# alphacep/vosk-tts

Hardware: NVIDIA H100
Metric: audio samples/sec @22.05kHz, 128-phoneme utterance (higher is better)
Workload: dtype fp32 (flow/decoder convs + attention: bf16 hi+lo split x3 MMAs on wgmma, fp32 accumulate; rest fp32 FFMA)

## Files before the change

### vosk_tts_b200/csrc/conv_tc.cuh

```cuda
#pragma once
#include <type_traits>
#include <cuda.h>
#include <cuda_bf16.h>
#include <cuda_runtime.h>
#include <stdint.h>
#include "wgmma.cuh"

namespace vtts {

constexpr int TC_BM = 128;
constexpr int TC_BK = 64;
#ifndef VTTS_TC_AST64
#define VTTS_TC_AST64 3
#endif
#ifndef VTTS_TC_WST64
#define VTTS_TC_WST64 4
#endif
#ifndef VTTS_TC_AST128
#define VTTS_TC_AST128 3
#endif
#ifndef VTTS_TC_WST128
#define VTTS_TC_WST128 4
#endif
template <int BN> constexpr int tc_ast() { return BN == 64 ? VTTS_TC_AST64 : VTTS_TC_AST128; }
template <int BN> constexpr int tc_wst() { return BN == 64 ? VTTS_TC_WST64 : VTTS_TC_WST128; }
constexpr int TC_CWG = 2;
constexpr int TC_THREADS = TC_CWG * 128 + 32;
constexpr int TC_MAXP = 4;

enum : int { TCE_RELU = 1, TCE_GATE = 2 };

struct TcProblemBase {
  CUtensorMap a_hi, a_lo, w_hi, w_lo;
  __nv_bfloat16* p_mid;
  const float* bias;
  const float* cond;
  const float* res;
  float* y;
  __nv_bfloat16* p_hi;
  __nv_bfloat16* p_lo;
  int cond_ld, ldr, roff, ldy, yoff, ldp, poff;
  int Cin, Cout, k, dil, pad;
  int out_mul, out_add;
  int in_extra, out_seq_extra;
  int epi;
  float alpha, pl_slope;
  int split;
  int cl0;
};
struct TcProblem : TcProblemBase {
  CUtensorMap a_mid, w_mid;
};

struct TcBatchScalars {
  int n;
  int rmul;
  int tall;
  int a_bytes;
  int baseoff;
  int cn;
  int wpre;
  int np;
  int ast, wst;
  int dbgskip;
  int wmc;
  int persist;
  int gx, gy, gz;
  int split;
  int mixed;
  int nb;
  unsigned long long* dbg;
};
template <class PT, int MP = TC_MAXP>
struct TcBatchT : TcBatchScalars {
  PT p[MP];
};
using TcBatch = TcBatchT<TcProblem>;
template <int MP>
inline TcBatchT<TcProblemBase, MP> tc_lite(const TcBatch& tb) {
  TcBatchT<TcProblemBase, MP> l;
  static_cast<TcBatchScalars&>(l) = tb;
  for (int i = 0; i < MP; ++i) l.p[i] = tb.p[i];
  return l;
}
__device__ __forceinline__ unsigned long long gtimer() {
  unsigned long long t;
  asm volatile("mov.u64 %0, %globaltimer;" : "=l"(t));
  return t;
}
#define TC_STAMP(i) do { if (tb.dbg && blockIdx.x == 0 && blockIdx.y == 0 && blockIdx.z == 0) tb.dbg[i] = gtimer(); } while (0)

__device__ __forceinline__ void tma_load_2d(void* dst, const CUtensorMap* map, int c0, int c1, uint64_t* bar) {
  asm volatile(
      "cp.async.bulk.tensor.2d.shared::cluster.global.mbarrier::complete_tx::bytes [%0], [%1, {%3, %4}], [%2];" ::"r"(smem_u32(dst)),
      "l"(reinterpret_cast<uint64_t>(map)), "r"(smem_u32(bar)), "r"(c0), "r"(c1)
      : "memory");
}
__device__ __forceinline__ void tma_load_2d_mc(void* dst, const CUtensorMap* map, int c0, int c1, uint64_t* bar, uint16_t mask) {
  asm volatile(
      "cp.async.bulk.tensor.2d.shared::cluster.global.mbarrier::complete_tx::bytes.multicast::cluster [%0], [%1, {%3, %4}], [%2], %5;" ::"r"(
          smem_u32(dst)),
      "l"(reinterpret_cast<uint64_t>(map)), "r"(smem_u32(bar)), "r"(c0), "r"(c1), "h"(mask)
      : "memory");
}
__device__ __forceinline__ uint32_t cluster_rank() {
  uint32_t r;
  asm volatile("mov.u32 %0, %%cluster_ctarank;" : "=r"(r));
  return r;
}
__device__ __forceinline__ void mbar_arrive_remote(uint64_t* bar, uint32_t rank) {
  uint32_t ra;
  asm volatile("mapa.shared::cluster.u32 %0, %1, %2;" : "=r"(ra) : "r"(smem_u32(bar)), "r"(rank));
  asm volatile("mbarrier.arrive.release.cluster.shared::cluster.b64 _, [%0];" ::"r"(ra) : "memory");
}
__device__ __forceinline__ void tc_release(uint64_t* bar, int n) {
  if (n > 1) {
    for (int r = 0; r < n; ++r) mbar_arrive_remote(bar, (uint32_t)r);
  } else {
    mbar_arrive(bar);
  }
}

__device__ __forceinline__ float tc_bias(const TcProblemBase& P, int b, int c) {
  float bv = P.bias[c];
  if (P.cond) bv += P.cond[(long)b * P.cond_ld + c];
  return bv;
}
__device__ __forceinline__ void tc_epi_pair(const TcProblemBase& P, int b, long orow, int c, float v0, float v1, int dbgskip) {
  const bool gate = (P.epi & TCE_GATE) != 0;
  float u[2];
  int oc, nout;
  if (gate) {
    oc = c >> 1;
    if (oc >= (P.Cout >> 1)) return;
    nout = 1;
    const float a = v0 + tc_bias(P, b, c), s = v1 + tc_bias(P, b, c + 1);
    u[0] = tanhf(a) * (1.f / (1.f + expf(-s)));
    u[1] = 0.f;
  } else {
    oc = c;
    if (oc >= P.Cout) return;
    nout = min(2, P.Cout - oc);
    u[0] = v0 + tc_bias(P, b, c);
    u[1] = nout > 1 ? v1 + tc_bias(P, b, c + 1) : 0.f;
  }
  const bool relu = (P.epi & TCE_RELU) != 0;
#pragma unroll
  for (int e = 0; e < 2; ++e) {
    float q = u[e];
    if (relu) q = fmaxf(q, 0.f);
    u[e] = q * P.alpha;
  }
  if (P.res && !(dbgskip & 4)) {
    const float* rp = P.res + orow * (long)P.ldr + P.roff + oc;
    if (nout == 2 && ((P.ldr | P.roff | oc) & 1) == 0) {
      const float2 q2 = *reinterpret_cast<const float2*>(rp);
      u[0] += q2.x; u[1] += q2.y;
    } else {
      for (int e = 0; e < nout; ++e) u[e] += rp[e];
    }
  }
  if (dbgskip & 1) return;
  if (P.y) {
    float* yr = P.y + orow * (long)P.ldy + P.yoff + oc;
    if (nout == 2 && ((P.ldy | P.yoff | oc) & 1) == 0) *reinterpret_cast<float2*>(yr) = make_float2(u[0], u[1]);
    else for (int e = 0; e < nout; ++e) yr[e] = u[e];
  }
  if (P.p_hi) {
    const long po = orow * (long)P.ldp + P.poff + oc;
    __align__(4) __nv_bfloat16 hb[2], mb[2], lb[2];
#pragma unroll
    for (int e = 0; e < 2; ++e) {
      float q = u[e];
      q = q > 0.f ? q : q * P.pl_slope;
      if (P.p_mid) split_bf16_3(q, hb[e], mb[e], lb[e]);
      else split_bf16(q, hb[e], lb[e]);
    }
    if (nout == 2 && ((P.ldp | P.poff | oc) & 1) == 0) {
      *reinterpret_cast<uint32_t*>(P.p_hi + po) = *reinterpret_cast<const uint32_t*>(hb);
      *reinterpret_cast<uint32_t*>(P.p_lo + po) = *reinterpret_cast<const uint32_t*>(lb);
      if (P.p_mid) *reinterpret_cast<uint32_t*>(P.p_mid + po) = *reinterpret_cast<const uint32_t*>(mb);
    } else {
      for (int e = 0; e < nout; ++e) {
        P.p_hi[po + e] = hb[e]; P.p_lo[po + e] = lb[e];
        if (P.p_mid) P.p_mid[po + e] = mb[e];
      }
    }
  }
}

template <int BN>
constexpr int tc_smem_bytes(int a_bytes, int np = 2, int ast = tc_ast<BN>(), int wst = tc_wst<BN>()) {
  return ast * np * a_bytes + wst * np * BN * TC_BK * 2 + 1024  + 256 ;
}
constexpr int TC_MAXST = 4;

struct TcTile {
  int pi;
  int b, co0, t0, sp;
  int s;
  int t0u;
  bool valid;
};

template <int BN, bool MIXED, class PT, int MP>
__device__ __forceinline__ void conv_tc_body(const TcBatchT<PT, MP>& tb, const int* __restrict__ lens, const int* __restrict__ offs) {
  constexpr bool HAS_MID = std::is_same<PT, TcProblem>::value;
  constexpr int B_BYTES = BN * TC_BK * 2;
  constexpr int NACC = BN / 2;
  const int TC_AST = tb.ast, TC_WST = tb.wst, NP = HAS_MID ? tb.np : 2;
  PDL_LAUNCH();
  if (threadIdx.x == 0) TC_STAMP(0);
  const int S = tb.split;
  const bool persist = tb.persist != 0;
  const int A_BYTES = tb.a_bytes;
  const bool tall = tb.tall != 0;
  const int wmc = persist ? tb.wmc : 1;
  const uint32_t wrank = wmc > 1 ? cluster_rank() : 0u;
  const int gxu = (tb.gx + wmc - 1) / wmc;
  const int ntiles = persist ? gxu * tb.gy * tb.gz : 1;
  const int tstride = persist ? (int)gridDim.x / wmc : 1;
  const int tile0 = persist ? (int)blockIdx.x / wmc : 0;
  auto decode_mixed = [&](int g) {
    const int ci = (int)blockIdx.z / S, rank = (int)blockIdx.z - ci * S;
    int pi = 0;
    while (pi + 1 < tb.n && ci >= tb.p[pi + 1].cl0) ++pi;
    const int s = tb.p[pi].split, gyp = (tb.p[pi].Cout + BN - 1) / BN;
    if (g < 0) g = rank / s;
    const int tile = (ci - tb.p[pi].cl0) * (S / s) + g;
    TcTile t;
    t.pi = pi;
    t.s = s;
    t.sp = rank % s;
    t.t0 = (tile % tb.gx) * TC_BM;
    t.t0u = t.t0;
    t.co0 = ((tile / tb.gx) % gyp) * BN;
    t.b = tile / (tb.gx * gyp);
    t.valid = t.b < tb.nb;
    return t;
  };
  auto decode = [&](int tile) {
    if constexpr (MIXED) { if (tb.mixed) return decode_mixed(-1); }
    int bx, by, bz, bxu;
    if (persist) {
      bxu = tile % gxu;
      const int r = tile / gxu;
      by = r % tb.gy;
      bz = r / tb.gy;
      bx = bxu * wmc + (int)wrank;
    } else {
      bx = blockIdx.x; by = blockIdx.y; bz = blockIdx.z;
      bxu = bx;
    }
    TcTile t;
    t.t0u = bxu * wmc * TC_BM;
    const int zi = bz / S;
    t.s = S;
    t.sp = bz - zi * S;
    t.pi = zi % tb.n;
    t.b = zi / tb.n;
    t.co0 = by * BN;
    t.t0 = bx * TC_BM;
    t.valid = t.co0 < tb.p[t.pi].Cout;
    return t;
  };

  extern __shared__ uint8_t tc_smem_raw[];
  uint8_t* smem = reinterpret_cast<uint8_t*>((reinterpret_cast<uintptr_t>(tc_smem_raw) + 1023) & ~(uintptr_t)1023);
  uint8_t* smem_w = smem + TC_AST * NP * A_BYTES;
  uint64_t* a_full = reinterpret_cast<uint64_t*>(smem_w + TC_WST * NP * B_BYTES);
  uint64_t* a_empty = a_full + TC_MAXST;
  uint64_t* w_full = a_empty + TC_MAXST;
  uint64_t* w_empty = w_full + TC_MAXST;

  const int warp = threadIdx.x >> 5, lane = threadIdx.x & 31;
  const bool producer = warp == TC_CWG * 4;
  const TcTile first = decode(tile0);
  const int cn = tb.cn;

  if (producer && lane == 0) {
    for (int s = 0; s < TC_AST; ++s) { mbar_init(&a_full[s], 1); mbar_init(&a_empty[s], (uint32_t)(cn * TC_CWG)); }
    for (int s = 0; s < TC_WST; ++s) { mbar_init(&w_full[s], 1); mbar_init(&w_empty[s], (uint32_t)(wmc * TC_CWG)); }
    asm volatile("fence.mbarrier_init.release.cluster;" ::: "memory");
    for (int q = 0; q < (persist ? tb.n : 1); ++q) {
      const PT& Q = tb.p[persist ? q : first.pi];
      asm volatile("prefetch.tensormap [%0];" ::"l"(reinterpret_cast<uint64_t>(&Q.a_hi)) : "memory");
      asm volatile("prefetch.tensormap [%0];" ::"l"(reinterpret_cast<uint64_t>(&Q.a_lo)) : "memory");
      asm volatile("prefetch.tensormap [%0];" ::"l"(reinterpret_cast<uint64_t>(&Q.w_hi)) : "memory");
      asm volatile("prefetch.tensormap [%0];" ::"l"(reinterpret_cast<uint64_t>(&Q.w_lo)) : "memory");
      if constexpr (HAS_MID) {
        if (NP == 3) {
          asm volatile("prefetch.tensormap [%0];" ::"l"(reinterpret_cast<uint64_t>(&Q.a_mid)) : "memory");
          asm volatile("prefetch.tensormap [%0];" ::"l"(reinterpret_cast<uint64_t>(&Q.w_mid)) : "memory");
        }
      }
    }
  }
  __syncthreads();
  const uint32_t crank = cn > 1 ? cluster_rank() : 0u;
  const uint16_t cmask = (uint16_t)((1u << cn) - 1u);
  if (cn > 1 || wmc > 1) cluster_sync_all();
  int w_pre = 0;
  auto issue_w = [&](const PT& P, int co0, int c, int j, int wst) {
    uint8_t* wb = smem_w + wst * NP * B_BYTES;
    mbar_expect_tx(&w_full[wst], NP * B_BYTES);
    if (wmc > 1) {
      const int half = (int)wrank * (BN / 2);
      tma_load_2d_mc(wb + half * 128, &P.w_hi, c * TC_BK, j * P.Cout + co0 + half, &w_full[wst], (uint16_t)3);
      tma_load_2d_mc(wb + B_BYTES + half * 128, &P.w_lo, c * TC_BK, j * P.Cout + co0 + half, &w_full[wst], (uint16_t)3);
      return;
    }
    tma_load_2d(wb, &P.w_hi, c * TC_BK, j * P.Cout + co0, &w_full[wst]);
    tma_load_2d(wb + B_BYTES, &P.w_lo, c * TC_BK, j * P.Cout + co0, &w_full[wst]);
    if constexpr (HAS_MID) { if (NP == 3) tma_load_2d(wb + 2 * B_BYTES, &P.w_mid, c * TC_BK, j * P.Cout + co0, &w_full[wst]); }
  };
  if (!persist && first.valid) {
    const PT& P = tb.p[first.pi];
    const int nsteps_all = (P.Cin / TC_BK) * P.k;
    const int s_beg = (int)((long)nsteps_all * first.sp / first.s), s_end = (int)((long)nsteps_all * (first.sp + 1) / first.s);
    const bool peek_active = first.t0 < lens[first.b] * tb.rmul + P.in_extra;
    w_pre = (tb.wpre && peek_active) ? min(TC_WST, s_end - s_beg) : 0;
    if (producer && lane == 0) {
      int c = s_beg / P.k, j = s_beg - c * P.k;
      for (int i = 0; i < w_pre; ++i) {
        issue_w(P, first.co0, c, j, i);
        if (++j == P.k) { j = 0; ++c; }
      }
    }
  }
  PDL_WAIT();
  if (threadIdx.x == 0) TC_STAMP(1);
  bool any_active = false;

  if (producer) {
    if (lane == 0) {
      int ast = 0, a_use = 0, wst = 0, w_use = 0;
      for (int tile = tile0; tile < ntiles; tile += tstride) {
        const TcTile T = persist ? decode(tile) : first;
        if (!T.valid) continue;
        const PT& P = tb.p[T.pi];
        const int L = lens[T.b] * tb.rmul + P.in_extra;
        if (T.t0u >= L) {
          for (int i = 0; i < w_pre; ++i) mbar_wait(&w_full[i], 0);
          continue;
        }
        any_active = true;
        const long in_base = (long)offs[T.b] * tb.rmul + (long)T.b * P.in_extra;
        const int nsteps_all = (P.Cin / TC_BK) * P.k;
        const int s_beg = (int)((long)nsteps_all * T.sp / T.s), s_end = (int)((long)nsteps_all * (T.sp + 1) / T.s);
        const int a_per = tall ? P.k : 1;
        const uint32_t a_tx = (uint32_t)NP * (uint32_t)(tall ? (TC_BM + (P.k - 1) * P.dil) : TC_BM) * 128u;
        int c = s_beg / P.k, j = s_beg - c * P.k;
        int a_cnt = 0;
        for (int s = s_beg; s < s_end; ++s) {
          const int ls = s - s_beg;
          if (a_cnt == 0) {
            if (a_use > 0) mbar_wait(&a_empty[ast], (a_use - 1) & 1);
            uint8_t* ab = smem + ast * NP * A_BYTES;
            mbar_expect_tx(&a_full[ast], a_tx);
            const int row = (int)in_base + T.t0 - P.pad + (tall ? 0 : j * P.dil);
            if (cn > 1) {
              const int slice = TC_BM / cn;
              const int soff = (int)crank * slice;
              tma_load_2d_mc(ab + soff * 128, &P.a_hi, c * TC_BK, row + soff, &a_full[ast], cmask);
              tma_load_2d_mc(ab + A_BYTES + soff * 128, &P.a_lo, c * TC_BK, row + soff, &a_full[ast], cmask);
            } else {
              tma_load_2d(ab, &P.a_hi, c * TC_BK, row, &a_full[ast]);
              tma_load_2d(ab + A_BYTES, &P.a_lo, c * TC_BK, row, &a_full[ast]);
              if constexpr (HAS_MID) { if (NP == 3) tma_load_2d(ab + 2 * A_BYTES, &P.a_mid, c * TC_BK, row, &a_full[ast]); }
            }
            if (++ast == TC_AST) { ast = 0; ++a_use; }
          }
          if (++a_cnt == a_per) a_cnt = 0;
          if (ls >= w_pre) {
            if (w_use > 0) mbar_wait(&w_empty[wst], (w_use - 1) & 1);
            issue_w(P, T.co0, c, j, wst);
          }
          if (++wst == TC_WST) { wst = 0; ++w_use; }
          if (++j == P.k) { j = 0; ++c; }
          if (ls == 0) TC_STAMP(2);
        }
        w_pre = 0;
        TC_STAMP(3);
      }
    }
    any_active = __shfl_sync(0xffffffffu, (int)any_active, 0) != 0;
  } else {
    const int wg = warp >> 2;
    const int g = lane >> 2, q4 = lane & 3;
    const int rbase = wg * 64 + (warp & 3) * 16 + g;
    const bool leader = (threadIdx.x & 127) == 0;
    int ast = 0, a_use = 0, wst = 0, w_use = 0;
    for (int tile = tile0; tile < ntiles; tile += tstride) {
      const TcTile T = persist ? decode(tile) : first;
      if (!T.valid) continue;
      const PT& P = tb.p[T.pi];
      const int L = lens[T.b] * tb.rmul + P.in_extra;
      if (T.t0u >= L) continue;
      any_active = true;
      const int nsteps_all = (P.Cin / TC_BK) * P.k;
      const int s_beg = (int)((long)nsteps_all * T.sp / T.s), s_end = (int)((long)nsteps_all * (T.sp + 1) / T.s);
      const int a_per = tall ? P.k : 1;
      float acc[NACC];
#pragma unroll
      for (int i = 0; i < NACC; ++i) acc[i] = 0.f;
      int j = s_beg % P.k;
      int a_cnt = 0;
      int prev_w = -1, prev_a = -1;
      for (int s = s_beg; s < s_end; ++s) {
        const int ls = s - s_beg;
        if (a_cnt == 0) mbar_wait(&a_full[ast], a_use & 1);
        mbar_wait(&w_full[wst], w_use & 1);
        if (ls == 0 && threadIdx.x == 0) TC_STAMP(4);
        const uint32_t abase = smem_u32(smem + ast * NP * A_BYTES) + (uint32_t)(wg * 64 * 128) + (tall ? (uint32_t)(j * P.dil) * 128u : 0u);
        const uint32_t wbase = smem_u32(smem_w + wst * NP * B_BYTES);
        const uint64_t ahi = gmma_desc_sw128(abase, tb.baseoff), alo = gmma_desc_sw128(abase + A_BYTES, tb.baseoff);
        const uint64_t bhi = gmma_desc_sw128(wbase), blo = gmma_desc_sw128(wbase + B_BYTES);
        auto mma = [&](uint64_t da, uint64_t db) {
          if constexpr (BN == 128) wgmma_ss_n128(acc, da, db);
          else wgmma_ss_n64(acc, da, db);
        };
        wgmma_fence();
        if (tb.dbgskip & 2) {
        } else if (NP == 3) {
          const uint64_t ami = gmma_desc_sw128(abase + 2 * A_BYTES, tb.baseoff), bmi = gmma_desc_sw128(wbase + 2 * B_BYTES);
#pragma unroll
          for (int kk = 0; kk < TC_BK / 16; ++kk) {
            const uint64_t adv = (uint64_t)((kk * 32) >> 4);
            mma(ahi + adv, blo + adv);
            mma(alo + adv, bhi + adv);
            mma(ami + adv, bmi + adv);
            mma(ami + adv, bhi + adv);
            mma(ahi + adv, bmi + adv);
            mma(ahi + adv, bhi + adv);
          }
        } else {
#pragma unroll
          for (int kk = 0; kk < TC_BK / 16; ++kk) {
            const uint64_t adv = (uint64_t)((kk * 32) >> 4);
            mma(alo + adv, bhi + adv);
            mma(ahi + adv, blo + adv);
            mma(ahi + adv, bhi + adv);
          }
        }
        wgmma_commit();
        wgmma_wait<1>();
        wgmma_touch<NACC>(acc);
        if (leader) {
          if (prev_w >= 0) tc_release(&w_empty[prev_w], wmc);
          if (prev_a >= 0) tc_release(&a_empty[prev_a], cn);
        }
        prev_w = wst;
        prev_a = -1;
        if (++wst == TC_WST) { wst = 0; ++w_use; }
        if (++a_cnt == a_per) {
          prev_a = ast;
          a_cnt = 0;
          if (++ast == TC_AST) { ast = 0; ++a_use; }
        }
        if (++j == P.k) j = 0;
      }
      wgmma_wait<0>();
      wgmma_touch<NACC>(acc);
      if (leader) {
        if (prev_w >= 0) tc_release(&w_empty[prev_w], wmc);
        if (prev_a >= 0) tc_release(&a_empty[prev_a], cn);
      }
      if (threadIdx.x == 0) TC_STAMP(5);
      const int b = T.b, co0 = T.co0;
      const long out_base = (long)offs[b] * tb.rmul * P.out_mul + (long)b * P.out_seq_extra;
      long orow[2];
      bool rowok[2];
#pragma unroll
      for (int h = 0; h < 2; ++h) {
        const int t = T.t0 + rbase + 8 * h;
        rowok[h] = t < L;
        orow[h] = out_base + (long)t * P.out_mul + P.out_add;
      }
      if (T.s == 1) {
#pragma unroll
        for (int jn = 0; jn < BN / 8; ++jn) {
          const int c = co0 + jn * 8 + 2 * q4;
#pragma unroll
          for (int h = 0; h < 2; ++h)
            if (rowok[h]) tc_epi_pair(P, b, orow[h], c, acc[4 * jn + 2 * h], acc[4 * jn + 2 * h + 1], tb.dbgskip);
        }
      } else {
        const int W = BN / T.s, sp = T.sp, g0 = MIXED ? (int)blockIdx.z % S - sp : 0;
        float* stage = reinterpret_cast<float*>(smem);
        cluster_sync_all();
#pragma unroll
        for (int jn = 0; jn < BN / 8; ++jn) {
          const int cc = jn * 8 + 2 * q4;
          const int qo = cc / W;
#pragma unroll
          for (int h = 0; h < 2; ++h) {
            uint32_t ra;
            asm volatile("mapa.shared::cluster.u32 %0, %1, %2;" : "=r"(ra) : "r"(smem_u32(stage + ((size_t)sp * TC_BM + rbase + 8 * h) * W + (cc - qo * W))), "r"(g0 + qo));
            asm volatile("st.shared::cluster.v2.f32 [%0], {%1, %2};" ::"r"(ra), "f"(acc[4 * jn + 2 * h]), "f"(acc[4 * jn + 2 * h + 1]) : "memory");
          }
        }
        cluster_sync_all();
#pragma unroll 1
        for (int u = 0; u < W / 4; ++u) {
          const int cw = 2 * q4 + 8 * (u >> 1), row = rbase + 8 * (u & 1), t = T.t0 + row;
          float v0 = 0.f, v1 = 0.f;
          for (int src = 0; src < T.s; ++src) {
            const float2 p2 = *reinterpret_cast<const float2*>(stage + ((size_t)src * TC_BM + row) * W + cw);
            v0 += p2.x; v1 += p2.y;
          }
          if (t < L) tc_epi_pair(P, b, out_base + (long)t * P.out_mul + P.out_add, co0 + sp * W + cw, v0, v1, tb.dbgskip);
        }
      }
    }
  }
  if (first.s > 1) {
    bool cl_active = any_active;
    if (MIXED && tb.mixed)
      for (int g = 0; g < S / first.s; ++g) {
        const TcTile u = decode_mixed(g);
        if (u.valid && u.t0 < lens[u.b] * tb.rmul + tb.p[u.pi].in_extra) cl_active = true;
      }
    if (cl_active && (producer || !any_active)) {
      __syncwarp();
      cluster_sync_all();
      cluster_sync_all();
    }
  }
  if (threadIdx.x == 0) TC_STAMP(7);
  __syncthreads();
  if (cn > 1 || wmc > 1) cluster_sync_all();
  if (threadIdx.x == 0) TC_STAMP(8);
}

template <int BN, bool DYN, int MP = TC_MAXP>
__global__ void __launch_bounds__(TC_THREADS, 1)
conv_tc_kernel(const __grid_constant__ TcBatchT<std::conditional_t<DYN, TcProblem, TcProblemBase>, MP> tb, const int* __restrict__ lens,
               const int* __restrict__ offs) {
  conv_tc_body<BN, true>(tb, lens, offs);
}
template <int BN>
__global__ void __launch_bounds__(TC_THREADS, 1)
conv_tc_persist_kernel(const __grid_constant__ TcBatch tb, const int* __restrict__ lens, const int* __restrict__ offs) {
  conv_tc_body<BN, false>(tb, lens, offs);
}

constexpr int EW_THREADS = 256;
constexpr int EW_ROWS = 16;

__global__ void __launch_bounds__(EW_THREADS)
split_planes_kernel(const float* __restrict__ x, int ldx, __nv_bfloat16* __restrict__ hi, __nv_bfloat16* __restrict__ lo,
                    int ldp, int C, float slope, int reflect, int rmul, const int* __restrict__ lens,
                    const int* __restrict__ offs) {
  PDL_LAUNCH();
  PDL_WAIT();
  const int b = blockIdx.y;
  const int Lphys = lens[b] * rmul;
  const int L = Lphys + (reflect ? 1 : 0);
  const int p0 = blockIdx.x * EW_ROWS;
  if (p0 >= L) return;
  const int nq = C >> 2;
  const int nrow = min(EW_ROWS, L - p0);
  const long base = (long)offs[b] * rmul;
  for (int u = threadIdx.x; u < nrow * nq; u += EW_THREADS) {
    const int r = u / nq, c = (u - r * nq) << 2;
    const int p = p0 + r;
    const int pr = reflect ? (p == 0 ? 1 : p - 1) : p;
    const long irow = base + pr;
    const long orow = base + (reflect ? b : 0) + p;
    const float4 v = *reinterpret_cast<const float4*>(x + irow * ldx + c);
    const float f[4] = {v.x, v.y, v.z, v.w};
    __align__(8) __nv_bfloat16 hb[4], lb[4];
#pragma unroll
    for (int i = 0; i < 4; ++i) {
      const float q = f[i] > 0.f ? f[i] : f[i] * slope;
      split_bf16(q, hb[i], lb[i]);
    }
    *reinterpret_cast<uint2*>(hi + orow * ldp + c) = *reinterpret_cast<const uint2*>(hb);
    *reinterpret_cast<uint2*>(lo + orow * ldp + c) = *reinterpret_cast<const uint2*>(lb);
  }
}

__global__ void __launch_bounds__(EW_THREADS)
mrf_mean_planes_kernel(const float* __restrict__ a, const float* __restrict__ b2, const float* __restrict__ c3, int n,
                       float* __restrict__ out, __nv_bfloat16* __restrict__ hi, __nv_bfloat16* __restrict__ lo, int C,
                       float slope, int reflect, int rmul, const int* __restrict__ lens, const int* __restrict__ offs) {
  PDL_LAUNCH();
  PDL_WAIT();
  const int b = blockIdx.y;
  const int Lphys = lens[b] * rmul;
  const int L = Lphys + (reflect ? 1 : 0);
  const int p0 = blockIdx.x * EW_ROWS;
  if (p0 >= L) return;
  const int nq = C >> 2;
  const int nrow = min(EW_ROWS, L - p0);
  const long base = (long)offs[b] * rmul;
  const float d = (float)n;
  for (int u = threadIdx.x; u < nrow * nq; u += EW_THREADS) {
    const int r = u / nq, c = (u - r * nq) << 2;
    const int p = p0 + r;
    const int pr = reflect ? (p == 0 ? 1 : p - 1) : p;
    const long irow = base + pr;
    const long orow = base + (reflect ? b : 0) + p;
    float4 s = *reinterpret_cast<const float4*>(a + irow * C + c);
    if (n > 1) { const float4 q = *reinterpret_cast<const float4*>(b2 + irow * C + c); s.x += q.x; s.y += q.y; s.z += q.z; s.w += q.w; }
    if (n > 2) { const float4 q = *reinterpret_cast<const float4*>(c3 + irow * C + c); s.x += q.x; s.y += q.y; s.z += q.z; s.w += q.w; }
    s.x /= d; s.y /= d; s.z /= d; s.w /= d;
    if (out && (!reflect || p >= 1)) *reinterpret_cast<float4*>(out + irow * C + c) = s;
    const float f[4] = {s.x, s.y, s.z, s.w};
    __align__(8) __nv_bfloat16 hb[4], lb[4];
#pragma unroll
    for (int i = 0; i < 4; ++i) {
      const float q = f[i] > 0.f ? f[i] : f[i] * slope;
      split_bf16(q, hb[i], lb[i]);
    }
    *reinterpret_cast<uint2*>(hi + orow * C + c) = *reinterpret_cast<const uint2*>(hb);
    *reinterpret_cast<uint2*>(lo + orow * C + c) = *reinterpret_cast<const uint2*>(lb);
  }
}

}
```

Measured before the change: 17.38 million.

## Prefetch epilogue bias/residual loads and overlap them with final wgmma wait

The epilogue is restructured around a precomputed TcEpi descriptor and per-column loads. Bias, cond and residual values for the first column are issued before the final wgmma wait, and each later column's inputs are prefetched one step ahead so global-load latency overlaps compute and stores. The split (s==1) and cluster-reduction paths now share one column loop, which walks columns by shifting the accumulator array each iteration. This adds register pressure and runtime-indexed or non-unrolled loops (unroll 1) that may cost instruction overhead.

```diff
diff --git a/vosk_tts_b200/csrc/conv_tc.cuh b/vosk_tts_b200/csrc/conv_tc.cuh
--- a/vosk_tts_b200/csrc/conv_tc.cuh
+++ b/vosk_tts_b200/csrc/conv_tc.cuh
@@ -121,69 +121,128 @@
   }
 }
 
-__device__ __forceinline__ float tc_bias(const TcProblemBase& P, int b, int c) {
-  float bv = P.bias[c];
-  if (P.cond) bv += P.cond[(long)b * P.cond_ld + c];
-  return bv;
-}
-__device__ __forceinline__ void tc_epi_pair(const TcProblemBase& P, int b, long orow, int c, float v0, float v1, int dbgskip) {
-  const bool gate = (P.epi & TCE_GATE) != 0;
+
+struct TcEpi {
+  const float* bias;
+  const float* cond;
+  const float* res;
+  float* y;
+  __nv_bfloat16 *p_hi, *p_lo, *p_mid;
+  int ldr, roff, ldy, yoff, ldp, poff;
+  int ncol;
+  float alpha, pl_slope;
+  bool gate, relu, store;
+};
+template <class PT>
+__device__ __forceinline__ TcEpi tc_epi(const PT& P, int b, int dbgskip) {
+  TcEpi E;
+  E.bias = P.bias;
+  E.cond = P.cond ? P.cond + (long)b * P.cond_ld : nullptr;
+  E.res = (dbgskip & 4) ? nullptr : P.res;
+  E.y = P.y;
+  E.p_hi = P.p_hi; E.p_lo = P.p_lo; E.p_mid = P.p_mid;
+  E.ldr = P.ldr; E.roff = P.roff; E.ldy = P.ldy; E.yoff = P.yoff; E.ldp = P.ldp; E.poff = P.poff;
+  E.gate = (P.epi & TCE_GATE) != 0;
+  E.relu = (P.epi & TCE_RELU) != 0;
+  E.ncol = E.gate ? P.Cout >> 1 : P.Cout;
+  E.alpha = P.alpha; E.pl_slope = P.pl_slope;
+  E.store = !(dbgskip & 1);
+  return E;
+}
+struct TcEpiCol {
+  int c, oc, nout;
+  bool ok;
+};
+__device__ __forceinline__ TcEpiCol tc_epi_col(const TcEpi& E, int c, bool in_tile) {
+  TcEpiCol k;
+  k.c = c;
+  k.oc = E.gate ? c >> 1 : c;
+  k.ok = in_tile && k.oc < E.ncol;
+  k.nout = E.gate ? 1 : min(2, E.ncol - k.oc);
+  return k;
+}
+struct TcEpiIn {
+  float b0, b1, c0, c1, r[2][2];
+};
+__device__ __forceinline__ TcEpiIn tc_epi_load(const TcEpi& E, const TcEpiCol& k, const long (&orow)[2], const bool (&rowok)[2]) {
+  TcEpiIn in = {};
+  if (!(k.ok && (rowok[0] || rowok[1]))) return in;
+  const bool two = E.gate || k.nout > 1;
+  in.b0 = E.bias[k.c];
+  if (two) in.b1 = E.bias[k.c + 1];
+  if (E.cond) {
+    in.c0 = E.cond[k.c];
+    if (two) in.c1 = E.cond[k.c + 1];
+  }
+  if (E.res) {
+#pragma unroll
+    for (int h = 0; h < 2; ++h) {
+      if (!rowok[h]) continue;
+      const float* rp = E.res + orow[h] * (long)E.ldr + E.roff + k.oc;
+      if (k.nout == 2 && ((E.ldr | E.roff | k.oc) & 1) == 0) {
+        const float2 q2 = *reinterpret_cast<const float2*>(rp);
+        in.r[h][0] = q2.x; in.r[h][1] = q2.y;
+      } else {
+        in.r[h][0] = rp[0];
+        if (k.nout > 1) in.r[h][1] = rp[1];
+      }
+    }
+  }
+  return in;
+}
+__device__ __forceinline__ void tc_epi_store(const TcEpi& E, const TcEpiCol& k, long orow, float b0, float b1, float c0, float c1,
+                                             float r0, float r1, float v0, float v1) {
+  const float bv0 = E.cond ? b0 + c0 : b0, bv1 = E.cond ? b1 + c1 : b1;
   float u[2];
-  int oc, nout;
-  if (gate) {
-    oc = c >> 1;
-    if (oc >= (P.Cout >> 1)) return;
-    nout = 1;
-    const float a = v0 + tc_bias(P, b, c), s = v1 + tc_bias(P, b, c + 1);
+  if (E.gate) {
+    const float a = v0 + bv0, s = v1 + bv1;
     u[0] = tanhf(a) * (1.f / (1.f + expf(-s)));
     u[1] = 0.f;
   } else {
-    oc = c;
-    if (oc >= P.Cout) return;
-    nout = min(2, P.Cout - oc);
-    u[0] = v0 + tc_bias(P, b, c);
-    u[1] = nout > 1 ? v1 + tc_bias(P, b, c + 1) : 0.f;
-  }
-  const bool relu = (P.epi & TCE_RELU) != 0;
+    u[0] = v0 + bv0;
+    u[1] = k.nout > 1 ? v1 + bv1 : 0.f;
+  }
 #pragma unroll
   for (int e = 0; e < 2; ++e) {
     float q = u[e];
-    if (relu) q = fmaxf(q, 0.f);
-    u[e] = q * P.alpha;
-  }
-  if (P.res && !(dbgskip & 4)) {
-    const float* rp = P.res + orow * (long)P.ldr + P.roff + oc;
-    if (nout == 2 && ((P.ldr | P.roff | oc) & 1) == 0) {
-      const float2 q2 = *reinterpret_cast<const float2*>(rp);
-      u[0] += q2.x; u[1] += q2.y;
+    if (E.relu) q = fmaxf(q, 0.f);
+    u[e] = __fmul_rn(q, E.alpha);
+  }
+  if (E.res) {
+    u[0] = __fadd_rn(u[0], r0);
+    if (k.nout > 1) u[1] = __fadd_rn(u[1], r1);
+  }
+  if (!E.store) return;
+  const int oc = k.oc, nout = k.nout;
+  if (E.y) {
+    float* yr = E.y + orow * (long)E.ldy + E.yoff + oc;
+    if (nout == 2 && ((E.ldy | E.yoff | oc) & 1) == 0) {
+      *reinterpret_cast<float2*>(yr) = make_float2(u[0], u[1]);
     } else {
-      for (int e = 0; e < nout; ++e) u[e] += rp[e];
-    }
-  }
-  if (dbgskip & 1) return;
-  if (P.y) {
-    float* yr = P.y + orow * (long)P.ldy + P.yoff + oc;
-    if (nout == 2 && ((P.ldy | P.yoff | oc) & 1) == 0) *reinterpret_cast<float2*>(yr) = make_float2(u[0], u[1]);
-    else for (int e = 0; e < nout; ++e) yr[e] = u[e];
-  }
-  if (P.p_hi) {
-    const long po = orow * (long)P.ldp + P.poff + oc;
-    __align__(4) __nv_bfloat16 hb[2], mb[2], lb[2];
+      yr[0] = u[0];
+      if (nout > 1) yr[1] = u[1];
+    }
+  }
+  if (E.p_hi) {
+    const long po = orow * (long)E.ldp + E.poff + oc;
+    __nv_bfloat16 hb[2], mb[2], lb[2];
 #pragma unroll
     for (int e = 0; e < 2; ++e) {
       float q = u[e];
-      q = q > 0.f ? q : q * P.pl_slope;
-      if (P.p_mid) split_bf16_3(q, hb[e], mb[e], lb[e]);
+      q = q > 0.f ? q : q * E.pl_slope;
+      if (E.p_mid) split_bf16_3(q, hb[e], mb[e], lb[e]);
       else split_bf16(q, hb[e], lb[e]);
     }
-    if (nout == 2 && ((P.ldp | P.poff | oc) & 1) == 0) {
-      *reinterpret_cast<uint32_t*>(P.p_hi + po) = *reinterpret_cast<const uint32_t*>(hb);
-      *reinterpret_cast<uint32_t*>(P.p_lo + po) = *reinterpret_cast<const uint32_t*>(lb);
-      if (P.p_mid) *reinterpret_cast<uint32_t*>(P.p_mid + po) = *reinterpret_cast<const uint32_t*>(mb);
+    if (nout == 2 && ((E.ldp | E.poff | oc) & 1) == 0) {
+      *reinterpret_cast<__nv_bfloat162*>(E.p_hi + po) = __halves2bfloat162(hb[0], hb[1]);
+      *reinterpret_cast<__nv_bfloat162*>(E.p_lo + po) = __halves2bfloat162(lb[0], lb[1]);
+      if (E.p_mid) *reinterpret_cast<__nv_bfloat162*>(E.p_mid + po) = __halves2bfloat162(mb[0], mb[1]);
     } else {
-      for (int e = 0; e < nout; ++e) {
-        P.p_hi[po + e] = hb[e]; P.p_lo[po + e] = lb[e];
-        if (P.p_mid) P.p_mid[po + e] = mb[e];
+      E.p_hi[po] = hb[0]; E.p_lo[po] = lb[0];
+      if (E.p_mid) E.p_mid[po] = mb[0];
+      if (nout > 1) {
+        E.p_hi[po + 1] = hb[1]; E.p_lo[po + 1] = lb[1];
+        if (E.p_mid) E.p_mid[po + 1] = mb[1];
       }
     }
   }
@@ -460,6 +519,22 @@
         }
         if (++j == P.k) j = 0;
       }
+      const int W = BN / T.s, ncp = W / 8;
+      const TcEpi E = tc_epi(P, T.b, tb.dbgskip);
+      const int cbase = T.co0 + T.sp * W + 2 * q4;
+      long orow[2];
+      bool rowok[2];
+      {
+        const long out_base = (long)offs[T.b] * tb.rmul * P.out_mul + (long)T.b * P.out_seq_extra;
+#pragma unroll
+        for (int h = 0; h < 2; ++h) {
+          const int t = T.t0 + rbase + 8 * h;
+          rowok[h] = t < L;
+          orow[h] = out_base + (long)t * P.out_mul + P.out_add;
+        }
+      }
+      auto col = [&](int j) { return tc_epi_col(E, cbase + 8 * j, j < ncp); };
+      TcEpiIn in = tc_epi_load(E, col(0), orow, rowok);
       wgmma_wait<0>();
       wgmma_touch<NACC>(acc);
       if (leader) {
@@ -467,27 +542,9 @@
         if (prev_a >= 0) tc_release(&a_empty[prev_a], cn);
       }
       if (threadIdx.x == 0) TC_STAMP(5);
-      const int b = T.b, co0 = T.co0;
-      const long out_base = (long)offs[b] * tb.rmul * P.out_mul + (long)b * P.out_seq_extra;
-      long orow[2];
-      bool rowok[2];
-#pragma unroll
-      for (int h = 0; h < 2; ++h) {
-        const int t = T.t0 + rbase + 8 * h;
-        rowok[h] = t < L;
-        orow[h] = out_base + (long)t * P.out_mul + P.out_add;
-      }
-      if (T.s == 1) {
-#pragma unroll
-        for (int jn = 0; jn < BN / 8; ++jn) {
-          const int c = co0 + jn * 8 + 2 * q4;
-#pragma unroll
-          for (int h = 0; h < 2; ++h)
-            if (rowok[h]) tc_epi_pair(P, b, orow[h], c, acc[4 * jn + 2 * h], acc[4 * jn + 2 * h + 1], tb.dbgskip);
-        }
-      } else {
-        const int W = BN / T.s, sp = T.sp, g0 = MIXED ? (int)blockIdx.z % S - sp : 0;
-        float* stage = reinterpret_cast<float*>(smem);
+      float* stage = reinterpret_cast<float*>(smem);
+      if (T.s > 1) {
+        const int sp = T.sp, g0 = MIXED ? (int)blockIdx.z % S - sp : 0;
         cluster_sync_all();
 #pragma unroll
         for (int jn = 0; jn < BN / 8; ++jn) {
@@ -501,16 +558,30 @@
           }
         }
         cluster_sync_all();
+      }
 #pragma unroll 1
-        for (int u = 0; u < W / 4; ++u) {
-          const int cw = 2 * q4 + 8 * (u >> 1), row = rbase + 8 * (u & 1), t = T.t0 + row;
-          float v0 = 0.f, v1 = 0.f;
-          for (int src = 0; src < T.s; ++src) {
-            const float2 p2 = *reinterpret_cast<const float2*>(stage + ((size_t)src * TC_BM + row) * W + cw);
-            v0 += p2.x; v1 += p2.y;
+      for (int j = 0; j < ncp; ++j) {
+        const TcEpiIn nx = tc_epi_load(E, col(j + 1), orow, rowok);
+        const TcEpiCol k = col(j);
+#pragma unroll 1
+        for (int h = 0; h < 2; ++h) {
+          if (!k.ok || !(h ? rowok[1] : rowok[0])) continue;
+          float v0 = h ? acc[2] : acc[0], v1 = h ? acc[3] : acc[1];
+          if (T.s > 1) {
+            const float* st = stage + (size_t)(rbase + 8 * h) * W + 8 * j + 2 * q4;
+            v0 = 0.f; v1 = 0.f;
+#pragma unroll 1
+            for (int src = 0; src < T.s; ++src) {
+              const float2 p2 = *reinterpret_cast<const float2*>(st + (size_t)src * TC_BM * W);
+              v0 += p2.x; v1 += p2.y;
+            }
           }
-          if (t < L) tc_epi_pair(P, b, out_base + (long)t * P.out_mul + P.out_add, co0 + sp * W + cw, v0, v1, tb.dbgskip);
-        }
+          tc_epi_store(E, k, h ? orow[1] : orow[0], in.b0, in.b1, in.c0, in.c1, h ? in.r[1][0] : in.r[0][0],
+                       h ? in.r[1][1] : in.r[0][1], v0, v1);
+        }
+#pragma unroll
+        for (int i = 0; i + 4 < NACC; ++i) acc[i] = acc[i + 4];
+        in = nx;
       }
     }
   }
```

After: 21.05 million (median of 6 runs). +21.1%, better.
